# TUMFTM/GraphBasedLocalTrajectoryPlanner

Measured on NVIDIA H100. Metric: planning ticks/s (10k-scenario batch, ~200x11 lattice), higher is better.
Workload: dtype f64 (decisions, splines, arc lengths) + f32 (velocity recurrences)

## Files before the change

graphbasedlocaltrajectoryplanner_b200/csrc/ltpl_api.cu:

```cuda
#include <atomic>
#include <cstddef>
#include <cstdio>
#include <cstdlib>
#include <cstring>
#include <mutex>
#include <new>
#include <string>

#include "ltpl_path.cuh"
#include "ltpl_plan.cuh"
#include "ltpl_vel.cuh"
#include "ltpl_vel_res.cuh"
#include "ltpl_velprofile.cuh"
#include "ltpl_emerg.cuh"
#include "ltpl_state.cuh"
#include "ltpl_smooth.cuh"

static std::atomic<unsigned long long> g_launches{0};

static thread_local std::string g_err;

static int fail(const char* what) {
    g_err = what;
    return -1;
// ... 366 lines not shown
                            void* stream) {
    if (int r = validate(lat, prm, dm, bf, false)) return r;
    cudaStream_t st = static_cast<cudaStream_t>(stream);
    if (bf->trim && bf->zone_s0 && cudaMemsetAsync(bf->zone_s0, 0xFF, sizeof(int) * (size_t)dm->batch, st) != cudaSuccess)
        return fail("memset(zone_s0) failed");
    k_startpos<<<ctas(dm->batch), kThreads, 0, st>>>(lat->d, *prm, *dm, *bf);
    return check_launch("k_startpos");
}

static int reset_counts(const LtplBuffers* bf, bool paths, cudaStream_t st) {
    const size_t n = paths ? 4 + 4 * LTPL_MAX_SUB : 1;
    if (cudaMemsetAsync(paths ? bf->queue_cnt : bf->queue_cnt + 2, 0, n * sizeof(int), st) != cudaSuccess)
        return fail("memset(queue_cnt) failed");
    return 0;
}

static int launch_export(const LtplDims* w, const LtplBuffers* bf, cudaStream_t st) {
    k_export<<<ctas(LTPL_NSLOT * w->sub_cnt, LTPL_WARPS_PER_CTA_EXPORT), LTPL_WARPS_PER_CTA_EXPORT * 32, 0, st>>>(*w, *bf);
    return check_launch("k_export");
}

static int launch_emergency(const LtplParams* prm, const LtplDims* w, const LtplBuffers* bf, cudaStream_t st) {
    const size_t smem = emerg_smem_bytes_per_warp(w->n_export) * LTPL_WARPS_PER_CTA;
    if (smem > 48 * 1024) return fail("n_export too large for k_emergency");
    k_emergency<<<ctas(w->sub_cnt), kThreads, smem, st>>>(*prm, *w, *bf);
    return check_launch("k_emergency");
}

static int launch_smooth(const LtplParams* prm, const LtplDims* w, const LtplBuffers* bf, cudaStream_t st, bool stateful) {
    const size_t smem = smooth_smem_bytes_per_warp(w->p_max) * LTPL_WARPS_PER_CTA;
    if (smem > 48 * 1024) return fail("dims.p_max too large for k_smooth");
    k_smooth<<<ctas(LTPL_NSLOT * w->sub_cnt), kThreads, smem, st>>>(*w, *bf, prm->filt_window, stateful ? 0 : 1);
    return check_launch("k_smooth");
}

static int paths_window(const LtplLattice* lat, const LtplParams* prm, const LtplDims* w, const LtplBuffers* bf,
                        cudaStream_t st, bool stateful) {
    if (stateful) {
        k_state<<<ctas(w->sub_cnt), kThreads, 0, st>>>(lat->d, *prm, *w, *bf);
        if (int r = check_launch("k_state")) return r;
    }
    if (int r = launch_k_plan(lat, prm, w, bf, st, stateful)) return r;
    return launch_k_path(lat, prm, w, bf, st, stateful);
}

static int vel_window(const LtplLattice* lat, const LtplParams* prm, const LtplDims* w, const LtplBuffers* bf,
                      cudaStream_t st, bool stateful) {
    const bool smooth = prm->filt_window > 1;
    if (stateful) {
        k_ref<<<ctas(w->sub_cnt), kThreads, 0, st>>>(lat->d, *prm, *w, *bf);
        if (int r = check_launch("k_ref")) return r;
    }
    if (int r = launch_k_vel(lat, prm, w, bf, st, stateful)) return r;
    if (stateful) {
        k_backup<<<ctas(w->sub_cnt), kThreads, 0, st>>>(*prm, *w, *bf);
        if (int r = check_launch("k_backup")) return r;
        k_prefix<<<ctas(LTPL_NSLOT * w->sub_cnt), kThreads, 0, st>>>(*w, *bf);
        if (int r = check_launch("k_prefix")) return r;
    }
    if (smooth)
        if (int r = launch_smooth(prm, w, bf, st, stateful)) return r;
    if (stateful)
        if (int r = launch_export(w, bf, st)) return r;
    if (prm->incl_emerg_traj) return launch_emergency(prm, w, bf, st);
    return 0;
}

enum { kPaths = 1, kVel = 2 };

static int run_tick(const LtplLattice* lat, const LtplParams* prm, const LtplDims* dm, const LtplBuffers* bf,
                    void* stream, int stages, bool stateful) {
    if (int r = validate(lat, prm, dm, bf, stateful)) return r;
    cudaStream_t st = static_cast<cudaStream_t>(stream);
    const bool paths = stages & kPaths, vel = stages & kVel, memory = bf->trim != nullptr;
    const size_t B = dm->batch;
    if (int r = reset_counts(bf, paths, st)) return r;
    if (memory && paths && !stateful && cudaMemsetAsync(bf->trim, 0, sizeof(int) * 4 * LTPL_NSLOT * B, st) != cudaSuccess)
        return fail("memset(trim) failed");
    if (memory && vel && !prm->incl_emerg_traj && bf->em_info &&
        cudaMemsetAsync(bf->em_info, 0xFF, sizeof(int) * 3 * B, st) != cudaSuccess)
        return fail("memset(em_info) failed");
    LtplBuffers vbf = *bf;
    if (stateful) vbf.vel = bf->vel_plan;
    return for_windows(lat, dm, st, [&](const LtplDims* w, cudaStream_t s) {
        if (paths)
            if (int r = paths_window(lat, prm, w, bf, s, stateful)) return r;
        return vel ? vel_window(lat, prm, w, &vbf, s, stateful) : 0;
    });
}

int ltpl_calc_paths_batch(const LtplLattice* lat, const LtplParams* prm, const LtplDims* dm, const LtplBuffers* bf,
                          void* stream) {
    return run_tick(lat, prm, dm, bf, stream, kPaths, false);
}

int ltpl_calc_vel_profile_batch(const LtplLattice* lat, const LtplParams* prm, const LtplDims* dm,
                                const LtplBuffers* bf, void* stream) {
    return run_tick(lat, prm, dm, bf, stream, kVel, false);
}

int ltpl_tick_batch(const LtplLattice* lat, const LtplParams* prm, const LtplDims* dm, const LtplBuffers* bf,
                    void* stream) {
    return run_tick(lat, prm, dm, bf, stream, kPaths | kVel, false);
}

int ltpl_next_calc_paths_batch(const LtplLattice* lat, const LtplParams* prm, const LtplDims* dm, const LtplBuffers* bf,
                               void* stream) {
    return run_tick(lat, prm, dm, bf, stream, kPaths, true);
}

int ltpl_next_calc_vel_profile_batch(const LtplLattice* lat, const LtplParams* prm, const LtplDims* dm,
                                     const LtplBuffers* bf, void* stream) {
    return run_tick(lat, prm, dm, bf, stream, kVel, true);
}

int ltpl_next_tick_batch(const LtplLattice* lat, const LtplParams* prm, const LtplDims* dm, const LtplBuffers* bf,
                         void* stream) {
    return run_tick(lat, prm, dm, bf, stream, kPaths | kVel, true);
}

int ltpl_launch_stage(int stage, const LtplLattice* lat, const LtplParams* prm, const LtplDims* dm,
                      const LtplBuffers* bf, void* stream) {
    if (int r = validate(lat, prm, dm, bf, false)) return r;
    cudaStream_t st = static_cast<cudaStream_t>(stream);
    const LtplDims w = window_dims(dm, 0, 1);
    switch (stage) {
        case 0: return ltpl_set_startpos_batch(lat, prm, dm, bf, stream);
        case 1: return launch_k_plan(lat, prm, &w, bf, st, false);
        case 2:
            if (int r = reset_counts(bf, true, st)) return r;
            return launch_k_path(lat, prm, &w, bf, st, false);
        case 3:
            if (int r = reset_counts(bf, false, st)) return r;
            return launch_k_vel(lat, prm, &w, bf, st, false);
        case 4: return launch_export(&w, bf, st);
        default: return fail("ltpl_launch_stage: unknown stage");
    }
}

int ltpl_velprofile_batch(const LtplParams* prm, const LtplVelBatch* vb, void* stream) {
    if (!prm || !vb) return fail("null argument");
    if (vb->n_paths <= 0 || vb->n_points < 2) return fail("velprofile: need n_paths > 0 and n_points >= 2");
    if (prm->n_axm < 1 || prm->n_axm > LTPL_MAX_AXM) return fail("params.n_axm out of range");
    if (prm->axm_v[prm->n_axm - 1] < prm->vel_max)
        return fail("ax_max_machines has to cover the entire velocity range of the car (i.e. >= v_max)!");
    if (prm->dyn_model_exp == 1.0)
        k_velprofile<true><<<(vb->n_paths + 31) / 32, 32, VD_SMEM_BYTES, static_cast<cudaStream_t>(stream)>>>(*prm, *vb);
    else
        k_velprofile<false><<<(vb->n_paths + 31) / 32, 32, VD_SMEM_BYTES, static_cast<cudaStream_t>(stream)>>>(*prm, *vb);
    return check_launch("k_velprofile");
}

#ifdef LTPL_PROFILE_PHASES
int ltpl_debug_phases(unsigned long long* out32, int reset) {
    if (out32) cudaMemcpyFromSymbol(out32, g_phase, sizeof(unsigned long long) * 32);
    if (reset) {
        unsigned long long z[32] = {0};
        cudaMemcpyToSymbol(g_phase, z, sizeof(z));
    }
    return 0;
}
#endif

}
```

graphbasedlocaltrajectoryplanner_b200/csrc/ltpl_common.cuh:

```cuda
#pragma once
#include <cuda_runtime.h>
#include <math_constants.h>
#include <stdint.h>

#include "ltpl_b200.h"

#ifdef LTPL_PROFILE_PHASES
__device__ unsigned long long g_phase[32];
#define LTPL_PH_INIT long long _t0 = clock64();
#define LTPL_PH(k)                                                                                   \
    {                                                                                                \
        long long _t1 = clock64();                                                                   \
        if ((threadIdx.x & 31) == 0) atomicAdd(&g_phase[k], (unsigned long long)(_t1 - _t0));        \
        _t0 = clock64();                                                                             \
    }
#else
#define LTPL_PH_INIT
#define LTPL_PH(k)
#endif

#define LTPL_FULL 0xffffffffu
#define LTPL_PI 3.141592653589793
#define LTPL_INF CUDART_INF

struct LatDev {
    int L, Nn, E, S, n_glob, closed, plan_mode, max_nodes, max_window_edges;
    double lat_offset, lat_res, step, vel_decrease_lat, veh_width, veh_length, virt_cost, min_plan_horizon;
    const int* node_off;
    const int* rl_idx;
    const double* s_rl;
    const double* vel_rl;
    const double2* refline;
    const double2* raceline;
    const double2* bound1;
    const double2* bound2;
    const double2* center;
    const double2* node_xy;
    const double* node_psi;
    const int* node_layer;
    const int2* in_off;
    const int* edge_layer_off;
    const int* edge_src;
    const int* edge_dst;
    const double* edge_cost;
    const double* edge_len;
    const double* edge_psi1;
    const double* edge_psi0;
    const int* samp_off;
    const double2* samp_xy;
    const double* samp_el;
    const int* samp_edge;
    const double* glob_rl;
    const double2* glob_xy;
    const LtplEdgeRec* edge_rec;
    const int* tab_reach;
    const unsigned char* tab_node;
    const int* tab_edge;
    int tab_stride;
    const int* grid_center;
    const int* grid_refline;
    const int* grid_raceline;
    const int* grid_glob;
    int grid_nx, grid_ny, grid_cyclic;
    double grid_x0, grid_y0, grid_inv_cell;
};

#ifndef LTPL_DEFAULT_SUB
#define LTPL_DEFAULT_SUB 4
#endif
#ifndef LTPL_SUB_MIN
#define LTPL_SUB_MIN 512
#endif
struct LtplLattice {
    LtplLatticeHeader h;
    LatDev d;
    int n_sub = 1, sub_min = LTPL_SUB_MIN;
    cudaStream_t aux[LTPL_MAX_SUB - 1] = {};
    cudaEvent_t ev_fork = nullptr, ev_join[LTPL_MAX_SUB - 1] = {};
    mutable size_t smem_allowed[4] = {};
    mutable int plan_carveout = -1;
};

__device__ __forceinline__ int sub_scenario(const LtplDims& dm, int warps_per_cta) {
    const int i = blockIdx.x * warps_per_cta + (threadIdx.x >> 5);
    return (i < dm.sub_cnt) ? dm.sub_off + i : -1;
}
__device__ __forceinline__ int sub_path(const LtplDims& dm, int warps_per_cta) {
    const int i = blockIdx.x * warps_per_cta + (threadIdx.x >> 5);
    if (i >= LTPL_NSLOT * dm.sub_cnt) return -1;
    return (i / dm.sub_cnt) * dm.batch + dm.sub_off + i % dm.sub_cnt;
}

__device__ __forceinline__ double sq_rn(double a) { return __dmul_rn(a, a); }

__device__ __forceinline__ double dist2_rn(double ax, double ay, double bx, double by) {
    return __dadd_rn(sq_rn(__dsub_rn(ax, bx)), sq_rn(__dsub_rn(ay, by)));
}

__device__ __forceinline__ double fast_rsqrt(double q) {
    double r = (double)rsqrtf((float)q);
    r = r * (1.5 - 0.5 * q * r * r);
    return r * (1.5 - 0.5 * q * r * r);
}
__device__ __forceinline__ double fast_rcp(double x) {
    double r = (double)__frcp_rn((float)x);
    r = r * (2.0 - x * r);
    return r * (2.0 - x * r);
}

__device__ __forceinline__ double angle3pt(double ax, double ay, double bx, double by, double cx, double cy) {
    double ang = atan2(cy - by, cx - bx) - atan2(ay - by, ax - bx);
    if (ang > LTPL_PI)
        ang -= 2 * LTPL_PI;
    else if (ang <= -LTPL_PI)
        ang += 2 * LTPL_PI;
    return ang;
}

struct AngCmp {
    bool gt, ge;
};
__device__ __noinline__ AngCmp angle_cmp_exact(double2 pn, double px, double py, double2 p1, double2 p2) {
    const double a1 = fabs(angle3pt(pn.x, pn.y, px, py, p1.x, p1.y));
    const double a2 = fabs(angle3pt(pn.x, pn.y, px, py, p2.x, p2.y));
    AngCmp r;
    r.gt = a1 > a2;
    r.ge = a1 >= a2;
    return r;
}
__device__ __forceinline__ AngCmp angle_cmp(double2 pn, double px, double py, double2 p1, double2 p2) {
    const double ux = pn.x - px, uy = pn.y - py;
    const double v1x = p1.x - px, v1y = p1.y - py, v2x = p2.x - px, v2y = p2.y - py;
    const double un = ux * ux + uy * uy, n1 = v1x * v1x + v1y * v1y, n2 = v2x * v2x + v2y * v2y;
    AngCmp r;
    if (un > 0.0 && n1 > 0.0 && n2 > 0.0) {
        const double c1 = (ux * v1x + uy * v1y) * fast_rsqrt(n1), c2 = (ux * v2x + uy * v2y) * fast_rsqrt(n2);
        const double d = c1 - c2;
        if (d * d > 1e-18 * un) {
            r.gt = r.ge = (c1 < c2);
            return r;
        }
    }
    return angle_cmp_exact(pn, px, py, p1, p2);
}

__device__ __forceinline__ double normalize_psi(double psi) {
    double a = fmod(fabs(psi), 2 * LTPL_PI);
    double out = (psi > 0.0) ? a : ((psi < 0.0) ? -a : 0.0);
    if (out >= LTPL_PI)
        out -= 2 * LTPL_PI;
    else if (out < -LTPL_PI)
        out += 2 * LTPL_PI;
    return out;
}

struct ArgMinD {
    double v;
    int i;
};

__device__ __forceinline__ ArgMinD warp_argmin(double v, int i) {
    const unsigned long long u = (unsigned long long)__double_as_longlong(v);
    const unsigned hi = (unsigned)(u >> 32), lo = (unsigned)u;
    const unsigned mh = __reduce_min_sync(LTPL_FULL, hi);
    const unsigned ml = __reduce_min_sync(LTPL_FULL, (hi == mh) ? lo : 0xffffffffu);
    const unsigned mi = __reduce_min_sync(LTPL_FULL, (hi == mh && lo == ml) ? (unsigned)i : 0xffffffffu);
    ArgMinD r;
    r.v = __longlong_as_double((long long)(((unsigned long long)mh << 32) | ml));
    r.i = (int)mi;
    return r;
}
// ... 219 lines not shown
```

graphbasedlocaltrajectoryplanner_b200/csrc/ltpl_vel_res.cuh:

```cuda
#pragma once
#include "ltpl_vel.cuh"

#ifndef VR_P
#define VR_P 8
#endif
#define VR_THREADS 64
#define VR_MAXM 16

__host__ __device__ inline size_t vr_smem_bytes(int nmax, bool gg) {
    return (size_t)VR_P * (gg ? 7 : 5) * nmax * sizeof(float);
}

__device__ __forceinline__ unsigned vr_s32(const void* p) { return (unsigned)__cvta_generic_to_shared(p); }
__device__ __forceinline__ void vr_mbar_init(unsigned long long* bar, unsigned count) {
    asm volatile("mbarrier.init.shared::cta.b64 [%0], %1;" ::"r"(vr_s32(bar)), "r"(count) : "memory");
    asm volatile("fence.mbarrier_init.release.cluster;" ::: "memory");
}
__device__ __forceinline__ void vr_mbar_expect_tx(unsigned long long* bar, unsigned bytes) {
    asm volatile("mbarrier.arrive.expect_tx.shared::cta.b64 _, [%0], %1;" ::"r"(vr_s32(bar)), "r"(bytes) : "memory");
}
__device__ __forceinline__ void vr_bulk_g2s(void* dst, const void* src, unsigned bytes, unsigned long long* bar) {
    asm volatile("cp.async.bulk.shared::cluster.global.mbarrier::complete_tx::bytes [%0], [%1], %2, [%3];" ::"r"(
                     vr_s32(dst)),
                 "l"(src), "r"(bytes), "r"(vr_s32(bar))
                 : "memory");
}
__device__ __forceinline__ void vr_mbar_wait(unsigned long long* bar, unsigned parity) {
    asm volatile(
        "{\n"
        ".reg .pred p;\n"
        "VR_WAIT:\n"
        "mbarrier.try_wait.parity.shared::cta.b64 p, [%0], %1;\n"
        "@p bra VR_DONE;\n"
        "bra VR_WAIT;\n"
        "VR_DONE:\n"
        "}\n" ::"r"(vr_s32(bar)),
        "r"(parity)
        : "memory");
}
__device__ __forceinline__ void vr_bar_arrive(int id) {
    __threadfence_block();
    asm volatile("bar.arrive %0, %1;" ::"r"(id), "r"(VR_THREADS) : "memory");
}
__device__ __forceinline__ void vr_bar_sync(int id) {
    asm volatile("bar.sync %0, %1;" ::"r"(id), "r"(VR_THREADS) : "memory");
}

#define VR_TAB (LTPL_MAX_AXM + 2)
struct VRCfg {
    float ax_max, dm, exp_, inv_exp;
    const float* xl;
    const float* x0;
    const float* f0;
    const float* sl;
    int n_seg;
};
__device__ __forceinline__ void vr_stage_axm(const LtplParams& prm, float* s_tab ) {
    const int n = prm.n_axm;
    for (int k = threadIdx.x; k <= n + 1; k += blockDim.x) {
        s_tab[k] = (k == 0) ? -CUDART_INF_F : ((k == n + 1) ? CUDART_INF_F : (float)prm.axm_v[k - 1]);
        if (k <= n) {
            const bool outer = (k == 0 || k == n);
            s_tab[VR_TAB + k] = outer ? 0.0f : (float)prm.axm_v[k - 1];
            s_tab[2 * VR_TAB + k] = (k == 0) ? (float)prm.axm_a[0] : (float)prm.axm_a[k - 1];
            s_tab[3 * VR_TAB + k] = outer ? 0.0f : (float)prm.axm_s[k - 1];
        }
    }
}
__device__ __forceinline__ VRCfg vr_make_cfg(const LtplParams& prm, const float* s_tab) {
    VRCfg c;
    c.ax_max = (float)(prm.gg_ax * prm.gg_scale);
    c.dm = (float)(prm.drag_coeff / prm.m_veh);
    c.exp_ = (float)prm.dyn_model_exp;
    c.inv_exp = (float)(1.0 / prm.dyn_model_exp);
    c.xl = s_tab;
    c.x0 = s_tab + VR_TAB;
    c.f0 = s_tab + 2 * VR_TAB;
    c.sl = s_tab + 3 * VR_TAB;
    c.n_seg = prm.n_axm + 1;
    return c;
}
__device__ __forceinline__ float vr_rcp(float x) {
    float y;
    asm("rcp.approx.ftz.f32 %0, %1;" : "=f"(y) : "f"(x));
    return y;
}
__device__ __forceinline__ float vr_sqrt(float x) {
    float y;
    asm("sqrt.approx.ftz.f32 %0, %1;" : "=f"(y) : "f"(x));
    return y;
}
__device__ __noinline__ float vr_tire_pow(float ratio, float ax_max, float e, float inv_e) {
    const float rad = 1.0f - powf(ratio, e);
    return (rad > 0.0f) ? ax_max * powf(rad, inv_e) : 0.0f;
}
template <bool EXP1>
__device__ __forceinline__ float vr_tire(const VRCfg& c, float w, float K, float ax) {
    if (EXP1) return ax * fmaxf(fmaf(-w, K, 1.0f), 0.0f);
    return vr_tire_pow(w * K, ax, c.exp_, c.inv_exp);
}

template <bool EXP1, bool GG>
__device__ __noinline__ void vr_forward(const VRCfg c, bool on, const float* __restrict__ K,
                                        const float* __restrict__ E2, const float* __restrict__ AX, float* __restrict__ W,
                                        int lo, int hi, float wcap, float we, float wmax, int nmax) {
    const int len = (on && hi >= lo) ? hi - lo : -1;
    int lmax = len;
#pragma unroll
    for (int o = 16; o > 0; o >>= 1) lmax = max(lmax, __shfl_xor_sync(LTPL_FULL, lmax, o));
    if (lmax < 0) return;
    if (len < 0) lo = 0;
    float k_prev = K[lo], ax_prev = GG ? AX[lo] : c.ax_max;
    float cur = fminf(fminf(vr_rcp(k_prev), wmax), wcap);
    if (len >= 0) W[lo] = cur;
    float o_prev = cur;
    bool prev_rise = false, active = false;
    int sg = 1;
    float xlo = c.xl[1], xhi = c.xl[2], x0 = c.x0[1], f0 = c.f0[1], sl = c.sl[1];
    const int pcap = nmax - 1;
#pragma unroll 2
    for (int i = 1; i <= lmax; ++i) {
        const bool live = i <= len;
        const int p = min(lo + i, pcap);
        const float kq = K[p], e2 = E2[p - 1];
        const float o_n = fminf(vr_rcp(kq), wmax);
        const bool rise = o_n > o_prev;
        active = active || (rise && !prev_rise);
        const float v = vr_sqrt(fmaxf(cur, 0.0f));
        const bool need = live && active;
        bool miss = need && !(v >= xlo && v < xhi);
        while (__any_sync(LTPL_FULL, miss)) {
            if (miss) sg += (v >= xhi) ? 1 : -1;
            xlo = c.xl[sg];
            xhi = c.xl[sg + 1];
            x0 = c.x0[sg];
            f0 = c.f0[sg];
            sl = c.sl[sg];
            miss = need && !(v >= xlo && v < xhi);
        }
        const float a_t = vr_tire<EXP1>(c, cur, k_prev, ax_prev);
        const float a_m = fmaf(sl, v - x0, f0);
        const float a = fmaf(-cur, c.dm, fminf(a_t, a_m));
        const float wn = fmaf(a, e2, cur);
        const float nxt = active ? fminf(wn, o_n) : o_n;
        active = active && !(wn > wmax);
        if (live) W[p] = nxt;
        cur = nxt;
        prev_rise = rise;
        o_prev = o_n;
        k_prev = kq;
        if (GG) ax_prev = AX[p];
    }
    if (len >= 0 && we >= 0.0f && W[hi] > we) W[hi] = we;
}
template <bool EXP1, bool GG>
__device__ __noinline__ void vr_brake(const VRCfg c, bool on, const float* __restrict__ K, const float* __restrict__ E2,
                                      const float* __restrict__ AX, float* __restrict__ W, int lo, int hi, float wcap,
                                      float we, int nmax) {
    const int len = (on && hi >= lo) ? hi - lo : -1;
    int lmax = len;
#pragma unroll
    for (int o = 16; o > 0; o >>= 1) lmax = max(lmax, __shfl_xor_sync(LTPL_FULL, lmax, o));
    if (lmax < 0) return;
    if (len < 0) lo = 0;
    float k_prev = K[lo], ax_prev = GG ? AX[lo] : c.ax_max;
    float cur = wcap;
    double cur64 = (double)cur;
    if (len >= 0) W[lo] = cur;
    const int pcap = nmax - 1;
#pragma unroll 2
    for (int i = 1; i <= lmax; ++i) {
        const int p = min(lo + i, pcap);
        const float kq = K[p], e2 = E2[p - 1];
        const float a = fmaf(-cur, c.dm, -vr_tire<EXP1>(c, cur, k_prev, ax_prev));
        cur64 = fmax(cur64 + (double)a * (double)e2, 0.0);
        cur = (float)cur64;
        if (i <= len) W[p] = cur;
        k_prev = kq;
        if (GG) ax_prev = AX[p];
    }
    if (len >= 0 && we >= 0.0f && W[hi] > we) W[hi] = we;
}
template <bool EXP1, bool GG>
__device__ __noinline__ float vr_backward(const VRCfg c, bool on, const float* __restrict__ K,
                                          const float* __restrict__ E2, const float* __restrict__ AX,
                                          const float* __restrict__ IAY, float* __restrict__ W, int lo, int hi,
                                          float wmax) {
    float cur = 0.0f;
    if (on && hi >= lo) {
        cur = W[hi];
        const int mir = lo + hi;
        float o_prev = cur;
        float k_p = GG ? K[hi] * vr_rcp(IAY[hi]) * IAY[mir - hi] : K[hi];
        float ax_p = GG ? AX[mir - hi] : c.ax_max;
        bool prev_rise = false, active = false;
#pragma unroll 2
        for (int p = hi - 1; p >= lo; --p) {
            const float o_n = W[p], e2 = E2[p];
            const float kq = GG ? K[p] * vr_rcp(IAY[p]) * IAY[mir - p] : K[p];
            const float axq = GG ? AX[mir - p] : c.ax_max;
            const bool rise = o_n > o_prev;
            active = active || (rise && !prev_rise);
            const float a = fmaf(cur, c.dm, vr_tire<EXP1>(c, cur, k_p, ax_p));
            float wn = fmaf(a, e2, cur);
            const float a2 = fmaf(wn, c.dm, vr_tire<EXP1>(c, wn, kq, axq));
            const float wt = fmaf(a2, e2, cur);
            wn = fminf(wn, wt);
            const float nxt = active ? fminf(wn, o_n) : o_n;
            active = active && !(wn > wmax);
            W[p] = nxt;
            cur = nxt;
            prev_rise = rise;
            o_prev = o_n;
            k_p = kq;
            ax_p = axq;
        }
    }
    return cur;
}

__device__ __forceinline__ int vr_first_ge_s(const float* __restrict__ S32, const double* __restrict__ sg, int n,
                                             double thr) {
    const float t = (float)thr;
    int lo = 0, hi = n;
    while (lo < hi) {
        const int mid = (lo + hi) >> 1;
        if (S32[mid] >= t)
            hi = mid;
        else
            lo = mid + 1;
    }
    while (lo < n && __ldcg(sg + lo) < thr) ++lo;
    return lo;
}
__device__ __forceinline__ int vr_first_le(const float* __restrict__ W, int n, float thr) {
    int lo = 0, hi = n;
    while (lo < hi) {
        const int mid = (lo + hi) >> 1;
        if (W[mid] <= thr)
            hi = mid;
        else
            lo = mid + 1;
    }
    return lo;
}

__device__ __forceinline__ double vr_s_coord_from_nb(const double* x, const double* y, const double* el, const double* sg,
                                                     int n, int nb, double px, double py) {
    const int idx1 = max(nb - 1, 0), idx2 = min(nb + 1, n - 1);
    const double xn = x[nb], yn = y[nb];
    int ia, ib;
    if (angle_cmp(make_double2(xn, yn), px, py, make_double2(x[idx1], y[idx1]), make_double2(x[idx2], y[idx2])).gt) {
        ia = idx1;
        ib = nb;
    } else {
        ia = nb;
        ib = idx2;
    }
    const bool ins = el[0] > 0.05;
    const double s_ia = __ldcg(sg + ia);
    const double sbase = ins ? s_ia : __dadd_rn(s_ia, el[ia]);
    const double ax = x[ia], ay = y[ia], bx = x[ib] - ax, by = y[ib] - ay;
    const double t = __ddiv_rn(__dadd_rn(__dmul_rn(px - ax, bx), __dmul_rn(py - ay, by)), __dadd_rn(sq_rn(bx), sq_rn(by)));
    const double sx = __dadd_rn(ax, __dmul_rn(t, bx)), sy = __dadd_rn(ay, __dmul_rn(t, by));
    const double ds = sqrt(__dadd_rn(sq_rn(ax - sx), sq_rn(ay - sy)));
    return __dadd_rn(sbase, ds);
}

__device__ __forceinline__ void vr_convert_kappa(float* X2, float* AX, float* IAY, int n, int sh, double inv_ay,
                                                 const double* gg_row, size_t gg_plane, double gg_scale, int lane) {
    const double* src = reinterpret_cast<const double*>(X2) + sh;
#pragma unroll 1
    for (int p0 = 0; p0 < n; p0 += 32) {
        const int p = p0 + lane;
        const double k = (p < n) ? src[p] : 0.0;
        double iay = inv_ay;
        if (gg_row && p < n) {
            iay = 1.0 / (gg_row[gg_plane + p] * gg_scale);
            AX[p] = (float)(gg_row[p] * gg_scale);
            IAY[p] = (float)iay;
        }
        __syncwarp();
        if (p < n) X2[p] = (float)(fabs(k) * iay);
    }
    __syncwarp();
}
#define VR_SC 6
__device__ __forceinline__ void vr_convert_el(float* X0, float* X4, double* s_out, int n, int sh, int lane) {
    const double* src = reinterpret_cast<const double*>(X0) + sh;
    double base = 0.0;
#pragma unroll 1
    for (int c0 = 0; c0 < n; c0 += 32 * VR_SC) {
        double e[VR_SC], inc[VR_SC];
#pragma unroll
        for (int j = 0; j < VR_SC; ++j) {
            const int p = c0 + 32 * j + lane;
            e[j] = (p < n) ? src[p] : 0.0;
            inc[j] = e[j];
        }
#pragma unroll
        for (int o = 1; o < 32; o <<= 1) {
#pragma unroll
            for (int j = 0; j < VR_SC; ++j) {
                const double v = __shfl_up_sync(LTPL_FULL, inc[j], o);
                if (lane >= o) inc[j] += v;
            }
        }
        __syncwarp();
#pragma unroll
        for (int j = 0; j < VR_SC; ++j) {
            const int p = c0 + 32 * j + lane;
            const double tot = __shfl_sync(LTPL_FULL, inc[j], 31);
            if (p < n) {
                const double sp = base + (inc[j] - e[j]);
                X0[p] = (float)(2.0 * e[j]);
                X4[p] = (float)sp;
                s_out[p] = sp;
            }
            base += tot;
        }
        __syncwarp();
    }
}

template <bool STATE, bool EXP1, bool GG>
__global__ void __launch_bounds__(VR_THREADS, 7)
k_vel_res(const LatDev lt, const LtplParams prm, const LtplDims dm, const LtplBuffers bf, const int nmax) {
    extern __shared__ __align__(16) unsigned char vr_smem[];
    __shared__ __align__(8) unsigned long long s_bar;
    __shared__ float s_tab[4 * VR_TAB];
    __shared__ int s_q[VR_P], s_n[VR_P], s_sh[VR_P], s_nb1[VR_P], s_nb2[VR_P], s_use_src[VR_P], s_row[VR_P], s_any_red;
    __shared__ long long s_in[VR_P], s_out[VR_P];
    __shared__ float s_wf0[VR_P], s_wcap[VR_P];
    __shared__ double s_v0[VR_P];
    const int tid = threadIdx.x, lane = tid & 31, warp = tid >> 5;
    const int B = dm.batch;
    const int nq = LTPL_NSLOT * B;
    const int nq_sub = LTPL_NSLOT * dm.sub_cnt;
    const int* queue = bf.queue + 2 * LTPL_NSLOT * dm.sub_off;
    const int n_follow = bf.queue_cnt[4 + 4 * dm.sub_id], n_other = bf.queue_cnt[4 + 4 * dm.sub_id + 1];
    const int gf = (n_follow + VR_P - 1) / VR_P, go = (n_other + VR_P - 1) / VR_P;
    const int g = blockIdx.x;
    if (g >= gf + go) return;
    const bool follow_cls = g < gf;
    const size_t pplane = (size_t)nq * dm.p_max;
    const double* x_pl = bf.path;
    const double* y_pl = bf.path + pplane;
    const double* k_pl = bf.path + 3 * pplane;
    const double* e_pl = bf.path + 4 * pplane;
    double* s_pl = bf.s_vx_ax;
    double* vx_pl = s_pl + pplane;
    double* ax_pl = vx_pl + pplane;

    if (tid == 0) s_any_red = 0;
    __syncthreads();
    if (tid < VR_P) {
        const int t = (follow_cls ? g : g - gf) * VR_P + tid;
        const bool live = t < (follow_cls ? n_follow : n_other);
        const int q = live ? queue[(follow_cls ? 0 : nq_sub) + t] : -1;
        int n = live ? bf.path_len[q] : 0;
        int off_in = 0, pref = 0;
        if (STATE && live) {
            pref = bf.trim[4 * q + 3];
            off_in = bf.trim[4 * q + 2] + pref;
            n = max(n - off_in, 0);
        }
        if (live && bf.vel[q % B] > prm.vel_max + 0.1) {
            atomicOr(&bf.sc_flags[q % B], LTPL_SC_BRAKE_PREFIX);
            n = 0;
        }
        if (n > nmax) {
            atomicOr(&bf.sc_flags[q % B], LTPL_SC_CAPACITY);
            n = 0;
        }
        const long long ib = (long long)max(q, 0) * dm.p_max + off_in;
        s_q[tid] = (n > 0) ? q : -1;
        s_n[tid] = n;
        s_in[tid] = ib;
        s_out[tid] = (long long)max(q, 0) * dm.p_max + pref;
        s_sh[tid] = (int)(ib & 1);
        s_use_src[tid] = 0;
        s_row[tid] = -1;
        s_wf0[tid] = 0.0f;
        if (follow_cls && n > 0 && (bf.status[q] & LTPL_ST_REDUCED_HORIZON)) s_any_red = 1;
    }
    vr_stage_axm(prm, s_tab);
    if (tid == 0) vr_mbar_init(&s_bar, 1);
    __syncthreads();
    int np = 0;
#pragma unroll
    for (int r = 0; r < VR_P; ++r) np = max(np, s_n[r]);
    if (np == 0) return;
    const bool any_red = s_any_red != 0;

    const size_t rowf = (size_t)(GG ? 7 : 5) * nmax;
    float* blk = reinterpret_cast<float*>(vr_smem);
    if (tid == 0) {
        unsigned total = 0;
        for (int r = 0; r < VR_P; ++r)
            if (s_n[r] > 0) total += 2u * 8u * (unsigned)((s_n[r] + s_sh[r] + 1) & ~1);
        vr_mbar_expect_tx(&s_bar, total);
        for (int r = 0; r < VR_P; ++r) {
            if (s_n[r] <= 0) continue;
            const unsigned bytes = 8u * (unsigned)((s_n[r] + s_sh[r] + 1) & ~1);
            float* X = blk + rowf * r;
            vr_bulk_g2s(X, e_pl + s_in[r] - s_sh[r], bytes, &s_bar);
            vr_bulk_g2s(X + 2 * (size_t)nmax, k_pl + s_in[r] - s_sh[r], bytes, &s_bar);
        }
    }
    const VRCfg c = vr_make_cfg(prm, s_tab);
    const float wmax = (float)(prm.vel_max * prm.vel_max);
    const double inv_ay = 1.0 / (prm.gg_ay * prm.gg_scale);
    const bool fw0 = follow_cls && warp == 0, fw1 = follow_cls && warp == 1;
    LTPL_PH_INIT

    const int pl = follow_cls ? lane % VR_P : min(2 * lane + warp, VR_P - 1);
    const bool lane_has = follow_cls ? (lane < VR_P) : (lane < VR_P / 2);
    const bool mine = lane_has && s_n[pl] > 0;
    const int q = s_q[pl], n = s_n[pl];
    const int b = mine ? q % B : 0;
    float* X = blk + rowf * pl;
    const float* E2 = X;
    float* WM = X + (size_t)nmax;
    const float* Kp = X + 2 * (size_t)nmax;
    float* SRC = X + 3 * (size_t)nmax;
    const float* S32 = X + 4 * (size_t)nmax;
    const float* AXp = X + 5 * (size_t)nmax;
    const float* IAYp = X + 6 * (size_t)nmax;
    const double* sg = s_pl + s_out[pl];
    const double vel_plan = mine ? bf.vel[b] : 0.0;
    const double vs_f = fmax(vel_plan, 0.0);
    const float wcap_m = (float)(vs_f * vs_f);
    if (mine) {
        s_wcap[pl] = wcap_m;
        s_v0[pl] = vs_f;
    }
    int st = mine ? bf.status[q] : 0;
    const int action = mine ? bf.action_id[q] : LTPL_ACT_NONE;
    const bool red = (st & LTPL_ST_REDUCED_HORIZON) != 0;
    bool vel_bound = true;

    const int ng = lt.n_glob - 1;
    const double* __restrict__ G = lt.glob_rl;
    const double ov = (fw1 && mine) ? bf.cobj[4 * b + 2] : 0.0;
    const int start = (fw1 && mine) ? bf.cobj_start[b] : 0;
    double opp_stop_dist = 0.0;
    if (fw1 && mine) {
        const double dmq = prm.drag_coeff / prm.m_veh;
        double v0 = fmin(ov, G[6 * start + 4]);
        if (v0 < 0.0) v0 = 0.0;
        double ww = v0 * v0;
        int id = 0;
        while (id < ng && ww > 0.01) {
            double e4[4], k4[4];
#pragma unroll
            for (int u = 0; u < 4; ++u) {
                int r = start + id + u;
                while (r >= ng) r -= ng;
                e4[u] = G[6 * r + 5];
                k4[u] = fabs(G[6 * r + 3]);
            }
#pragma unroll
            for (int u = 0; u < 4; ++u) {
                if (id < ng && ww > 0.01) {
                    opp_stop_dist += e4[u];
                    ++id;
                    if (id <= ng - 1) {
                        const double a = acc_brake(ww, k4[u], 14.0, 1.0 / 14.0, prm.dyn_model_exp, dmq);
                        const double nx = fma(2.0 * a, e4[u], ww);
                        ww = (nx < 0.0) ? 0.0 : nx;
                    } else {
                        ww = 0.0;
                    }
                }
            }
        }
    }
    LTPL_PH(6)

    vr_mbar_wait(&s_bar, 0);
    LTPL_PH(0)
    for (int r = follow_cls ? 0 : warp; r < VR_P; r += (follow_cls ? 1 : 2)) {
        const int nr = s_n[r];
        if (nr <= 0) continue;
        float* Xr = blk + rowf * r;
        if (!fw0)
            vr_convert_kappa(Xr + 2 * (size_t)nmax, Xr + 5 * (size_t)nmax, Xr + 6 * (size_t)nmax, nr, s_sh[r], inv_ay,
                             GG ? bf.gg + s_in[r] : nullptr, pplane, prm.gg_scale, lane);
        if (!fw1) vr_convert_el(Xr, Xr + 4 * (size_t)nmax, s_pl + s_out[r], nr, s_sh[r], lane);
    }
    LTPL_PH(1)
    if (fw1) {
        vr_bar_arrive(1);
        if (!STATE) {
            constexpr int LPP = 32 / VR_P;
            const int r = lane / LPP, sub = lane % LPP;
            const int nr = s_n[r];
            const int br = (nr > 0) ? s_q[r] % B : 0;
            const double ox = bf.cobj[4 * br], oy = bf.cobj[4 * br + 1];
            const double epx = bf.pos[2 * br], epy = bf.pos[2 * br + 1];
            const double* xr = x_pl + s_in[r];
            const double* yr = y_pl + s_in[r];
            double bv1 = LTPL_INF, bv2 = LTPL_INF;
            int i1 = 0x7fffffff, i2 = 0x7fffffff;
#pragma unroll 1
            for (int p0 = sub; p0 < nr; p0 += 8 * LPP) {
                double xx[8], yy[8];
#pragma unroll
                for (int u = 0; u < 8; ++u) {
                    const int p = min(p0 + u * LPP, nr - 1);
                    xx[u] = xr[p];
                    yy[u] = yr[p];
                }
#pragma unroll
                for (int u = 0; u < 8; ++u) {
                    const int p = p0 + u * LPP;
                    const double d1 = dist2_rn(xx[u], yy[u], ox, oy), d2 = dist2_rn(xx[u], yy[u], epx, epy);
                    if (p < nr && d1 < bv1) {
                        bv1 = d1;
                        i1 = p;
                    }
                    if (p < nr && d2 < bv2) {
                        bv2 = d2;
                        i2 = p;
                    }
                }
            }
#pragma unroll
            for (int o = 1; o < LPP; o <<= 1) {
                const double u1 = __shfl_xor_sync(LTPL_FULL, bv1, o), u2 = __shfl_xor_sync(LTPL_FULL, bv2, o);
                const int j1 = __shfl_xor_sync(LTPL_FULL, i1, o), j2 = __shfl_xor_sync(LTPL_FULL, i2, o);
                if (u1 < bv1 || (u1 == bv1 && j1 < i1)) {
                    bv1 = u1;
                    i1 = j1;
                }
                if (u2 < bv2 || (u2 == bv2 && j2 < i2)) {
                    bv2 = u2;
                    i2 = j2;
                }
            }
            if (sub == 0 && nr > 0) {
                s_nb1[r] = i1;
                s_nb2[r] = i2;
            }
            __syncwarp();
        }
        LTPL_PH(8)
    } else if (fw0) {
        vr_bar_arrive(2);
        vr_bar_sync(1);
    } else {
        __threadfence_block();
        __syncwarp();
    }

    int flags = 0, idx_c = 0, stop_idx = 0, hi = -1;
    bool use_prof = false, has_ctrl = false;
    double vcs = 0.0;
    const int rounds = follow_cls ? (any_red ? 3 : 2) : 1;
#pragma unroll 1
    for (int round = 0; round < rounds; ++round) {
        bool on = false;
        int lo = 0;
        float wcap = wcap_m, we = -1.0f, wmx = wmax;
        float* W = WM;
        bool brake = false;
        hi = -1;
        if (round == 2) {
            for (int r = 0; r < VR_P; ++r) {
                float* Wr = blk + rowf * r + nmax;
                const float* Sr = blk + rowf * r + 3 * (size_t)nmax;
                for (int p = tid; p < s_n[r]; p += VR_THREADS) Wr[p] = fminf(Sr[p], Wr[p]);
            }
            __syncthreads();
        }
        if (!follow_cls || (fw0 && round == 2)) {
            on = mine && (!follow_cls || red);
            if (on) {
                double v_end;
                int v_idx;
                if (red) {
                    v_end = 0.0;
                    const double spl_len = __ldcg(sg + n - 1);
                    int first = vr_first_ge_s(S32 + 1, sg + 1, n - 1, spl_len - 5.0);
                    if (first >= n - 1) first = 0;
                    v_idx = first + 1;
                    if (v_idx == 1 && n > 1) v_idx = n;
                } else {
                    const int nn = bf.n_nodes[q];
                    const int* nd = bf.nodes + ((size_t)q * dm.h_max + (nn - 1)) * 2;
                    const int end_layer = nd[0], end_node = nd[1];
                    int dn = end_node - lt.rl_idx[end_layer];
                    if (dn < 0) dn = -dn;
                    const double raceline_offset = dn * lt.lat_offset;
                    v_end = lt.vel_rl[end_layer];
                    v_end -= fmin(v_end * lt.vel_decrease_lat * raceline_offset, v_end);
                    v_idx = n;
                }
                if (v_idx > 1) {
                    hi = v_idx - 1;
                    const double ve = fmax(v_end, 0.0);
                    we = (float)(ve * ve);
                }
                if (follow_cls) W = SRC;
            }
        } else if (fw0 && round == 0) {
            on = mine;
            hi = n - 1;
        } else if (fw1 && round == 0) {
            LTPL_PH(7)
            vr_bar_sync(2);
            LTPL_PH(9)
            on = mine;
            brake = true;
            hi = n - 1;
            W = SRC;
        } else if (fw1 && round == 1) {
            double v_end_c = 0.0, v_control = 0.0;
            if (mine) {
                double obj_dist;
                if (STATE) {
                    obj_dist = bf.obj_dist[b];
                } else {
                    const double* xr = x_pl + s_in[pl];
                    const double* yr = y_pl + s_in[pl];
                    const double* er = e_pl + s_in[pl];
                    const double s_obj = vr_s_coord_from_nb(xr, yr, er, sg, n, s_nb1[pl], bf.cobj[4 * b], bf.cobj[4 * b + 1]);
                    const double s_start = vr_s_coord_from_nb(xr, yr, er, sg, n, s_nb2[pl], bf.pos[2 * b], bf.pos[2 * b + 1]);
                    obj_dist = s_obj - s_start;
                }
                const double v_ego = bf.vel_est[b];
                const double control_d = prm.follow_c_p * prm.safety_d + lt.veh_length;
                const double safety_d = prm.safety_d + lt.veh_length;
                if ((obj_dist - safety_d) < 0) flags |= 1;
                const int pz = vr_first_le(SRC, n, 0.01f);
                const double ego_stop_dist = (pz < n) ? __ldcg(sg + pz) : __ldcg(sg + n - 1) + (e_pl + s_in[pl])[n - 1];
                const double s_stop = obj_dist - safety_d + opp_stop_dist;
                stop_idx = min(vr_first_ge_s(S32, sg, n, s_stop), n - 1);
                const double s_last = __ldcg(sg + n - 1);
                if (s_stop > s_last) {
                    const double s_ends = opp_stop_dist - (s_stop - s_last);
                    int idx = 0;
                    double s_summed = 0.0;
                    while (s_summed < s_ends && idx < ng) {
                        double e4[4];
#pragma unroll
                        for (int u = 0; u < 4; ++u) {
                            int r4 = start + idx + u;
                            while (r4 >= ng) r4 -= ng;
                            e4[u] = G[6 * r4 + 5];
                        }
#pragma unroll
                        for (int u = 0; u < 4; ++u)
                            if (s_summed < s_ends && idx < ng) {
                                s_summed += e4[u];
                                ++idx;
                            }
                    }
                    int r = start + idx;
                    while (r >= ng) r -= ng;
                    v_end_c = G[6 * r + 4];
                }
                if (prm.follow_control_type == 0) {
                    v_control = ov - prm.follow_k_p * (control_d - obj_dist) + prm.follow_k_d * (ov - v_ego);
                } else {
                    double arg = (control_d - obj_dist) * LTPL_PI / 2 * 1 / prm.follow_tan_w;
                    arg = fmin(fmax(arg, -LTPL_PI / 2 + 1e-5), LTPL_PI / 2 - 1e-5);
                    v_control = ov - tan(arg) * prm.follow_k_p + prm.follow_k_d * (ov - v_ego);
                }
                v_control = fmin(fmax(v_control, 0.0), prm.vel_max);
                if (ego_stop_dist < s_stop) {
                    use_prof = true;
                    if (vel_plan > v_control && stop_idx >= 2) {
                        int first = vr_first_le(SRC, n, (float)(v_control * v_control));
                        if (first >= n) first = 0;
                        idx_c = min(first, stop_idx);
                        if (idx_c == 0) idx_c = stop_idx;
                        vcs = sqrt((double)SRC[idx_c]);
                    } else {
                        if (!(stop_idx >= 2)) flags |= 2;
                        idx_c = 0;
                        vcs = vel_plan;
                    }
                    has_ctrl = (stop_idx - idx_c) > 0;
                }
            }
            const double vcs_p = fmax(vcs, 0.0), vec_p = fmax(v_end_c, 0.0);
            on = mine && use_prof && has_ctrl;
            lo = idx_c;
            hi = on ? stop_idx : -1;
            wcap = (float)(vcs_p * vcs_p);
            we = (float)(vec_p * vec_p);
            wmx = (float)(v_control * v_control);
            W = SRC;
            LTPL_PH(10)
        }

        if (fw1 && round == 0) {
            vr_brake<EXP1, GG>(c, on, Kp, E2, AXp, W, lo, hi, wcap, we, nmax);
        } else {
            vr_forward<EXP1, GG>(c, on, Kp, E2, AXp, W, lo, hi, wcap, we, wmx, nmax);
            if (fw0 && round == 0) {
                LTPL_PH(3)
            }
        }
        const float w_first = vr_backward<EXP1, GG>(c, on && !brake, Kp, E2, AXp, IAYp, W, lo, hi, wmx);

        if (!follow_cls || (fw0 && round == 2)) {
            if (on) {
                for (int p = hi + 1; p < n; ++p) W[p] = 0.0f;
                const float wf0 = (hi >= 0) ? w_first : 0.0f;
                if (follow_cls) {
                    s_wf0[pl] = wf0;
                    s_use_src[pl] = (n >= 6 && !(WM[5] < SRC[5])) ? 1 : 0;
                } else {
                    vel_bound = fabs(sqrt((double)wf0) - vel_plan) < prm.v_max_offset;
                }
            }
        } else if (fw1 && round == 1) {
            if (mine && use_prof) {
                const double vcs_p = fmax(vcs, 0.0);
                if (!has_ctrl) SRC[idx_c] = (float)(vcs_p * vcs_p);
                for (int p = stop_idx + 1; p < n; ++p) SRC[p] = 0.0f;
                const double v0c = has_ctrl ? sqrt((double)w_first) : vcs;
                if (has_ctrl && fabs(v0c - vcs) > 1.0) flags |= 2;
                const double prof0 = (idx_c == 0) ? v0c : vs_f;
                if (fabs(prof0 - vel_plan) > 1.0) flags |= 2;
            }
            if (flags & 1) st |= LTPL_ST_TOO_CLOSE;
            vel_bound = !(flags & 2);
            LTPL_PH(11)
        } else if (fw0 && round == 0) {
            LTPL_PH(4)
        }
        if (follow_cls && round >= 1)
            __syncthreads();
        else
            __syncwarp();
        if (follow_cls && round == 1) {
            LTPL_PH(5 + 7 * warp)
        }
    }

    if (mine && !fw0) {
        if (follow_cls && red) vel_bound = fabs(sqrt((double)s_wf0[pl]) - vel_plan) < prm.v_max_offset;
        if (!vel_bound) st |= LTPL_ST_VEL_BOUND_VIOL;
        if (STATE && !vel_bound && (action == LTPL_ACT_FOLLOW || action == LTPL_ACT_STRAIGHT) && bf.const_len[b] != 0)
            atomicOr(&bf.sc_flags[b], LTPL_SC_STATE_FALLBACK | (6 << LTPL_SC_REASON_SHIFT));
        if (vel_bound || action == LTPL_ACT_FOLLOW || action == LTPL_ACT_STRAIGHT) {
            st |= LTPL_ST_TRAJ_VALID;
            bf.traj_len[q] = min(n, dm.n_export);
            bf.traj_id[q] = prm.traj_base_id + action;
            const int e = atomicAdd(&bf.queue_cnt[2], 1);
            bf.exp_q[e] = q;
            bf.traj_row[q] = e;
            s_row[pl] = e;
        }
        bf.status[q] = st;
    }
    if (follow_cls)
        __syncthreads();
    else
        __syncwarp();

    {
        const int t0 = follow_cls ? tid : lane, tstep = follow_cls ? VR_THREADS : 32;
        for (int r = follow_cls ? 0 : warp; r < VR_P; r += (follow_cls ? 1 : 2)) {
            const int nr = s_n[r];
            if (nr <= 0) continue;
            const float* Er = blk + rowf * r;
            const float* Wr = Er + nmax;
            const float* Sr = Er + 3 * (size_t)nmax;
            const float* S32r = Er + 4 * (size_t)nmax;
            const int mode = !follow_cls ? 1 : (any_red ? (s_use_src[r] ? 2 : 1) : 0);
            for (int p = t0; p < nr; p += tstep) {
                const float w0 = (mode == 0) ? fminf(Sr[p], Wr[p]) : ((mode == 1) ? Wr[p] : Sr[p]);
                float a = 0.0f;
                if (p < nr - 1) {
                    const float w1 = (mode == 0) ? fminf(Sr[p + 1], Wr[p + 1]) : ((mode == 1) ? Wr[p + 1] : Sr[p + 1]);
                    a = (w1 - w0) * vr_rcp(Er[p]);
                    if (w0 <= 1e-16f && fabsf(a) <= 1e-8f) a = -5.0f;
                }
                const double v = (p == 0 && w0 == s_wcap[r]) ? s_v0[r] : (double)sqrtf(w0);
                vx_pl[s_out[r] + p] = v;
                ax_pl[s_out[r] + p] = (double)a;
            }
            const int er = STATE ? -1 : s_row[r];
            const int ne = (er >= 0) ? min(nr, dm.n_export) : 0;
            float* __restrict__ out = bf.traj + (size_t)max(er, 0) * dm.n_export * 7;
            const double* __restrict__ ppr = bf.path + s_in[r];
#pragma unroll 1
            for (int p0 = t0; p0 < ne; p0 += 4 * tstep) {
                double g[4][4];
#pragma unroll
                for (int u = 0; u < 4; ++u) {
                    const int p = min(p0 + u * tstep, ne - 1);
#pragma unroll
                    for (int cc = 0; cc < 4; ++cc) g[u][cc] = ppr[cc * pplane + p];
                }
#pragma unroll
                for (int u = 0; u < 4; ++u) {
                    const int p = p0 + u * tstep;
                    if (p < ne) {
                        const float w0 = (mode == 0) ? fminf(Sr[p], Wr[p]) : ((mode == 1) ? Wr[p] : Sr[p]);
                        float a = 0.0f;
                        if (p < nr - 1) {
                            const float w1 = (mode == 0) ? fminf(Sr[p + 1], Wr[p + 1])
                                                         : ((mode == 1) ? Wr[p + 1] : Sr[p + 1]);
                            a = (w1 - w0) * vr_rcp(Er[p]);
                            if (w0 <= 1e-16f && fabsf(a) <= 1e-8f) a = -5.0f;
                        }
                        float* o = out + (size_t)p * 7;
                        o[0] = S32r[p];
                        o[1] = (float)g[u][0];
                        o[2] = (float)g[u][1];
                        o[3] = (float)g[u][2];
                        o[4] = (float)g[u][3];
                        o[5] = (p == 0 && w0 == s_wcap[r]) ? (float)s_v0[r] : sqrtf(w0);
                        o[6] = a;
                    }
                }
            }
        }
    }
    LTPL_PH(13)
}
```

Before: 25.53 million.

## Flatten trajectory export across rows, early-exit brake loop, widen nearest-point batch

The export loop now walks all exported rows as one flat index space. It prefetches the next four path points across row boundaries, so the global loads for the next batch overlap the stores of the current one. The brake recurrence exits early once every lane has reached zero velocity, then zero-fills the remaining entries cooperatively across the warp. The nearest-point search batch grows from 8 to 16 loads, and the per-phase and per-CTA profiling instrumentation is extended; it compiles out by default. The changes trade extra registers and control logic for fewer serial recurrence steps and better latency hiding.

```diff
diff --git a/graphbasedlocaltrajectoryplanner_b200/csrc/ltpl_api.cu b/graphbasedlocaltrajectoryplanner_b200/csrc/ltpl_api.cu
--- a/graphbasedlocaltrajectoryplanner_b200/csrc/ltpl_api.cu
+++ b/graphbasedlocaltrajectoryplanner_b200/csrc/ltpl_api.cu
@@ -542,13 +542,19 @@
 }
 
 #ifdef LTPL_PROFILE_PHASES
-int ltpl_debug_phases(unsigned long long* out32, int reset) {
-    if (out32) cudaMemcpyFromSymbol(out32, g_phase, sizeof(unsigned long long) * 32);
+int ltpl_debug_phases(unsigned long long* out64, unsigned long long* cta, int reset) {
+    unsigned n = 0;
+    cudaMemcpyFromSymbol(&n, g_cta_n, sizeof(n));
+    if (n > LTPL_PH_NCTA) n = LTPL_PH_NCTA;
+    if (out64) cudaMemcpyFromSymbol(out64, g_phase, sizeof(unsigned long long) * 64);
+    if (cta && n) cudaMemcpyFromSymbol(cta, g_cta, sizeof(unsigned long long) * n);
     if (reset) {
-        unsigned long long z[32] = {0};
+        unsigned long long z[64] = {0};
+        const unsigned zn = 0;
         cudaMemcpyToSymbol(g_phase, z, sizeof(z));
-    }
-    return 0;
+        cudaMemcpyToSymbol(g_cta_n, &zn, sizeof(zn));
+    }
+    return (int)n;
 }
 #endif
 
diff --git a/graphbasedlocaltrajectoryplanner_b200/csrc/ltpl_common.cuh b/graphbasedlocaltrajectoryplanner_b200/csrc/ltpl_common.cuh
--- a/graphbasedlocaltrajectoryplanner_b200/csrc/ltpl_common.cuh
+++ b/graphbasedlocaltrajectoryplanner_b200/csrc/ltpl_common.cuh
@@ -6,17 +6,36 @@
 #include "ltpl_b200.h"
 
 #ifdef LTPL_PROFILE_PHASES
-__device__ unsigned long long g_phase[32];
-#define LTPL_PH_INIT long long _t0 = clock64();
+#define LTPL_PH_NCTA 16384
+__device__ unsigned long long g_phase[64];
+__device__ unsigned long long g_cta[LTPL_PH_NCTA];
+__device__ unsigned int g_cta_n;
+#define LTPL_PH_INIT                                                                                 \
+    long long _t0 = clock64();                                                                       \
+    [[maybe_unused]] const long long _t_entry = _t0;                                                 \
+    int _ph_off = 0;
+#define LTPL_PH_CLASS(off) _ph_off = (off);
 #define LTPL_PH(k)                                                                                   \
     {                                                                                                \
         long long _t1 = clock64();                                                                   \
-        if ((threadIdx.x & 31) == 0) atomicAdd(&g_phase[k], (unsigned long long)(_t1 - _t0));        \
+        if ((threadIdx.x & 31) == 0) atomicAdd(&g_phase[(k) + _ph_off], (unsigned long long)(_t1 - _t0)); \
         _t0 = clock64();                                                                             \
+    }
+#define LTPL_PH_CTA(tag)                                                                             \
+    {                                                                                                \
+        __syncthreads();                                                                             \
+        if (threadIdx.x == 0) {                                                                      \
+            const unsigned long long _c = (unsigned long long)(clock64() - _t_entry);                \
+            atomicAdd(&g_phase[14 + _ph_off], _c);                                                   \
+            const unsigned _i = atomicAdd(&g_cta_n, 1u);                                             \
+            if (_i < LTPL_PH_NCTA) g_cta[_i] = (_c << 2) | (unsigned long long)(tag);                \
+        }                                                                                            \
     }
 #else
 #define LTPL_PH_INIT
+#define LTPL_PH_CLASS(off)
 #define LTPL_PH(k)
+#define LTPL_PH_CTA(tag)
 #endif
 
 #define LTPL_FULL 0xffffffffu
diff --git a/graphbasedlocaltrajectoryplanner_b200/csrc/ltpl_vel_res.cuh b/graphbasedlocaltrajectoryplanner_b200/csrc/ltpl_vel_res.cuh
--- a/graphbasedlocaltrajectoryplanner_b200/csrc/ltpl_vel_res.cuh
+++ b/graphbasedlocaltrajectoryplanner_b200/csrc/ltpl_vel_res.cuh
@@ -5,6 +5,7 @@
 #define VR_P 8
 #endif
 #define VR_THREADS 64
+#define VR_NB 16
 #define VR_MAXM 16
 
 __host__ __device__ inline size_t vr_smem_bytes(int nmax, bool gg) {
@@ -168,8 +169,10 @@
     double cur64 = (double)cur;
     if (len >= 0) W[lo] = cur;
     const int pcap = nmax - 1;
+    const bool can_stop = !GG && !(c.ax_max < 0.0f);
+    int i = 1;
 #pragma unroll 2
-    for (int i = 1; i <= lmax; ++i) {
+    for (; i <= lmax; ++i) {
         const int p = min(lo + i, pcap);
         const float kq = K[p], e2 = E2[p - 1];
         const float a = fmaf(-cur, c.dm, -vr_tire<EXP1>(c, cur, k_prev, ax_prev));
@@ -178,7 +181,21 @@
         if (i <= len) W[p] = cur;
         k_prev = kq;
         if (GG) ax_prev = AX[p];
-    }
+        if (can_stop && (i & 7) == 0 &&
+            __all_sync(LTPL_FULL, i >= len || __double_as_longlong(cur64) == 0)) {
+            ++i;
+            break;
+        }
+    }
+    unsigned rest = __ballot_sync(LTPL_FULL, i <= len);
+    while (rest) {
+        const int j = __ffs(rest) - 1;
+        rest &= rest - 1;
+        float* Wj = reinterpret_cast<float*>(__shfl_sync(LTPL_FULL, reinterpret_cast<unsigned long long>(W), j));
+        const int from = __shfl_sync(LTPL_FULL, lo + i, j), to = __shfl_sync(LTPL_FULL, hi, j);
+        for (int p = from + (threadIdx.x & 31); p <= to; p += 32) Wj[p] = 0.0f;
+    }
+    __syncwarp();
     if (len >= 0 && we >= 0.0f && W[hi] > we) W[hi] = we;
 }
 template <bool EXP1, bool GG>
@@ -323,6 +340,21 @@
     }
 }
 
+__device__ __forceinline__ int vr_end_mode(bool follow_cls, bool any_red, int use_src) {
+    return !follow_cls ? 1 : (any_red ? (use_src ? 2 : 1) : 0);
+}
+__device__ __forceinline__ void vr_end_point(const float* Er, int nmax, int mode, int n, int p, float& w0, float& a) {
+    const float* Wr = Er + nmax;
+    const float* Sr = Er + 3 * (size_t)nmax;
+    w0 = (mode == 0) ? fminf(Sr[p], Wr[p]) : ((mode == 1) ? Wr[p] : Sr[p]);
+    a = 0.0f;
+    if (p < n - 1) {
+        const float w1 = (mode == 0) ? fminf(Sr[p + 1], Wr[p + 1]) : ((mode == 1) ? Wr[p + 1] : Sr[p + 1]);
+        a = (w1 - w0) * vr_rcp(Er[p]);
+        if (w0 <= 1e-16f && fabsf(a) <= 1e-8f) a = -5.0f;
+    }
+}
+
 template <bool STATE, bool EXP1, bool GG>
 __global__ void __launch_bounds__(VR_THREADS, 7)
 k_vel_res(const LatDev lt, const LtplParams prm, const LtplDims dm, const LtplBuffers bf, const int nmax) {
@@ -333,6 +365,7 @@
     __shared__ long long s_in[VR_P], s_out[VR_P];
     __shared__ float s_wf0[VR_P], s_wcap[VR_P];
     __shared__ double s_v0[VR_P];
+    LTPL_PH_INIT
     const int tid = threadIdx.x, lane = tid & 31, warp = tid >> 5;
     const int B = dm.batch;
     const int nq = LTPL_NSLOT * B;
@@ -343,6 +376,7 @@
     const int g = blockIdx.x;
     if (g >= gf + go) return;
     const bool follow_cls = g < gf;
+    LTPL_PH_CLASS(follow_cls ? 0 : 32)
     const size_t pplane = (size_t)nq * dm.p_max;
     const double* x_pl = bf.path;
     const double* y_pl = bf.path + pplane;
@@ -412,7 +446,6 @@
     const float wmax = (float)(prm.vel_max * prm.vel_max);
     const double inv_ay = 1.0 / (prm.gg_ay * prm.gg_scale);
     const bool fw0 = follow_cls && warp == 0, fw1 = follow_cls && warp == 1;
-    LTPL_PH_INIT
 
     const int pl = follow_cls ? lane % VR_P : min(2 * lane + warp, VR_P - 1);
     const bool lane_has = follow_cls ? (lane < VR_P) : (lane < VR_P / 2);
@@ -504,16 +537,16 @@
             double bv1 = LTPL_INF, bv2 = LTPL_INF;
             int i1 = 0x7fffffff, i2 = 0x7fffffff;
 #pragma unroll 1
-            for (int p0 = sub; p0 < nr; p0 += 8 * LPP) {
-                double xx[8], yy[8];
-#pragma unroll
-                for (int u = 0; u < 8; ++u) {
+            for (int p0 = sub; p0 < nr; p0 += VR_NB * LPP) {
+                double xx[VR_NB], yy[VR_NB];
+#pragma unroll
+                for (int u = 0; u < VR_NB; ++u) {
                     const int p = min(p0 + u * LPP, nr - 1);
                     xx[u] = xr[p];
                     yy[u] = yr[p];
                 }
 #pragma unroll
-                for (int u = 0; u < 8; ++u) {
+                for (int u = 0; u < VR_NB; ++u) {
                     const int p = p0 + u * LPP;
                     const double d1 = dist2_rn(xx[u], yy[u], ox, oy), d2 = dist2_rn(xx[u], yy[u], epx, epy);
                     if (p < nr && d1 < bv1) {
@@ -698,6 +731,7 @@
 
         if (fw1 && round == 0) {
             vr_brake<EXP1, GG>(c, on, Kp, E2, AXp, W, lo, hi, wcap, we, nmax);
+            LTPL_PH(2)
         } else {
             vr_forward<EXP1, GG>(c, on, Kp, E2, AXp, W, lo, hi, wcap, we, wmx, nmax);
             if (fw0 && round == 0) {
@@ -762,56 +796,59 @@
         __syncthreads();
     else
         __syncwarp();
+    LTPL_PH(15)
 
     {
         const int t0 = follow_cls ? tid : lane, tstep = follow_cls ? VR_THREADS : 32;
-        for (int r = follow_cls ? 0 : warp; r < VR_P; r += (follow_cls ? 1 : 2)) {
+        const int r0 = follow_cls ? 0 : warp, rs = follow_cls ? 1 : 2;
+        int cr = r0, cb = 0;
+        double g[4][4];
+        int gr[4], gp[4];
+        auto ne_of = [&](int r) { return (!STATE && s_row[r] >= 0) ? min(s_n[r], dm.n_export) : 0; };
+        auto fetch = [&](int k0) {
+#pragma unroll
+            for (int u = 0; u < 4; ++u) {
+                const int k = k0 + u * tstep;
+                while (cr < VR_P && k >= cb + ne_of(cr)) {
+                    cb += ne_of(cr);
+                    cr += rs;
+                }
+                gr[u] = cr;
+                gp[u] = k - cb;
+                if (cr < VR_P) {
+                    const double* __restrict__ ppr = bf.path + s_in[cr] + gp[u];
+#pragma unroll
+                    for (int cc = 0; cc < 4; ++cc) g[u][cc] = ppr[cc * pplane];
+                }
+            }
+        };
+        if (!STATE) fetch(t0);
+        for (int r = r0; r < VR_P; r += rs) {
             const int nr = s_n[r];
             if (nr <= 0) continue;
             const float* Er = blk + rowf * r;
-            const float* Wr = Er + nmax;
-            const float* Sr = Er + 3 * (size_t)nmax;
-            const float* S32r = Er + 4 * (size_t)nmax;
-            const int mode = !follow_cls ? 1 : (any_red ? (s_use_src[r] ? 2 : 1) : 0);
+            const int mode = vr_end_mode(follow_cls, any_red, s_use_src[r]);
             for (int p = t0; p < nr; p += tstep) {
-                const float w0 = (mode == 0) ? fminf(Sr[p], Wr[p]) : ((mode == 1) ? Wr[p] : Sr[p]);
-                float a = 0.0f;
-                if (p < nr - 1) {
-                    const float w1 = (mode == 0) ? fminf(Sr[p + 1], Wr[p + 1]) : ((mode == 1) ? Wr[p + 1] : Sr[p + 1]);
-                    a = (w1 - w0) * vr_rcp(Er[p]);
-                    if (w0 <= 1e-16f && fabsf(a) <= 1e-8f) a = -5.0f;
-                }
+                float w0, a;
+                vr_end_point(Er, nmax, mode, nr, p, w0, a);
                 const double v = (p == 0 && w0 == s_wcap[r]) ? s_v0[r] : (double)sqrtf(w0);
                 vx_pl[s_out[r] + p] = v;
                 ax_pl[s_out[r] + p] = (double)a;
             }
-            const int er = STATE ? -1 : s_row[r];
-            const int ne = (er >= 0) ? min(nr, dm.n_export) : 0;
-            float* __restrict__ out = bf.traj + (size_t)max(er, 0) * dm.n_export * 7;
-            const double* __restrict__ ppr = bf.path + s_in[r];
+        }
+        LTPL_PH(23)
+        if (!STATE) {
 #pragma unroll 1
-            for (int p0 = t0; p0 < ne; p0 += 4 * tstep) {
-                double g[4][4];
+            for (int k0 = t0; gr[0] < VR_P;) {
 #pragma unroll
                 for (int u = 0; u < 4; ++u) {
-                    const int p = min(p0 + u * tstep, ne - 1);
-#pragma unroll
-                    for (int cc = 0; cc < 4; ++cc) g[u][cc] = ppr[cc * pplane + p];
-                }
-#pragma unroll
-                for (int u = 0; u < 4; ++u) {
-                    const int p = p0 + u * tstep;
-                    if (p < ne) {
-                        const float w0 = (mode == 0) ? fminf(Sr[p], Wr[p]) : ((mode == 1) ? Wr[p] : Sr[p]);
-                        float a = 0.0f;
-                        if (p < nr - 1) {
-                            const float w1 = (mode == 0) ? fminf(Sr[p + 1], Wr[p + 1])
-                                                         : ((mode == 1) ? Wr[p + 1] : Sr[p + 1]);
-                            a = (w1 - w0) * vr_rcp(Er[p]);
-                            if (w0 <= 1e-16f && fabsf(a) <= 1e-8f) a = -5.0f;
-                        }
-                        float* o = out + (size_t)p * 7;
-                        o[0] = S32r[p];
+                    const int r = gr[u], p = gp[u];
+                    if (r < VR_P) {
+                        const float* Er = blk + rowf * r;
+                        float w0, a;
+                        vr_end_point(Er, nmax, vr_end_mode(follow_cls, any_red, s_use_src[r]), s_n[r], p, w0, a);
+                        float* o = bf.traj + ((size_t)s_row[r] * dm.n_export + p) * 7;
+                        o[0] = Er[4 * (size_t)nmax + p];
                         o[1] = (float)g[u][0];
                         o[2] = (float)g[u][1];
                         o[3] = (float)g[u][2];
@@ -820,8 +857,11 @@
                         o[6] = a;
                     }
                 }
+                k0 += 4 * tstep;
+                fetch(k0);
             }
         }
     }
     LTPL_PH(13)
-}
+    LTPL_PH_CTA((any_red ? 2 : 0) | (follow_cls ? 1 : 0))
+}
```

Result: no change. 25.63 million (median of 6 runs) (+0.4%).
